# BlockstreamResearch/secp256k1-zkp

Measured on AMD Instinct MI355X. Metric: 64-bit Borromean rangeproof verifies/sec, higher is better.
Workload: dtype u32 limbs (9x29-bit), 32x32->64 integer MAC

## Files before the change

### __graft_entry__.py

```python
import os
import subprocess
import sys

ROOT = os.path.dirname(os.path.abspath(__file__))
CSRC = os.path.join(ROOT, "secp256k1_zkp_amd", "csrc")
HIPCC = os.environ.get("HIPCC", "/opt/rocm/bin/hipcc")
HIP_FLAGS = ["--offload-arch=gfx950", "-O3", "-std=c++17", "-shared", "-fPIC", "-Wno-unused-value"]


def _run(cmd, cwd=None):
    print("+", " ".join(cmd), flush=True)
    subprocess.check_call(cmd, cwd=cwd)


def _stale(target, sources):
    if not os.path.exists(target):
        return True
    t = os.path.getmtime(target)
    return any(os.path.getmtime(s) > t for s in sources if os.path.exists(s))


def build(force=False):
    hdrs = [os.path.join(CSRC, f) for f in os.listdir(CSRC) if f.endswith((".h", ".hip"))] + [os.path.join(ROOT, "include", "secp256k1_zkp_amd.h")]
    sys.path.insert(0, ROOT)
    from secp256k1_zkp_amd import build_lib
    build_lib.build(force=force)
    prims_src = os.path.join(ROOT, "tests", "gpu_prims", "prims.hip")
    prims = os.path.join(ROOT, "tests", "gpu_prims", "libs2k_gpuprims.so")
    if force or _stale(prims, hdrs + [prims_src]):
        _run([HIPCC] + HIP_FLAGS + ["-o", prims, prims_src])
    winv_src = os.path.join(ROOT, "tests", "wave_inverse", "waveinv_test.hip")
    winv = os.path.join(ROOT, "tests", "wave_inverse", "libs2k_waveinv_test.so")
    if force or _stale(winv, hdrs + [winv_src]):
        _run([HIPCC] + HIP_FLAGS + ["-o", winv, winv_src])
    wlanes_src = os.path.join(ROOT, "tests", "wave_inverse", "waveinv_lanes_test.hip")
    wlanes = os.path.join(ROOT, "tests", "wave_inverse", "libs2k_waveinv_lanes_test.so")
    if force or _stale(wlanes, hdrs + [wlanes_src]):
        _run([HIPCC] + HIP_FLAGS + ["-o", wlanes, wlanes_src])
    emu_src = os.path.join(ROOT, "tests", "host_emul", "hostemu.cpp")
    emu = os.path.join(ROOT, "tests", "host_emul", "libs2k_hostemu.so")
    if force or _stale(emu, hdrs + [emu_src]):
        _run(["g++", "-O2", "-std=c++17", "-fPIC", "-shared", "-o", emu, emu_src])
    ecdsa_emu_src = os.path.join(ROOT, "tests", "host_emul", "ecdsa_emu.cpp")
    ecdsa_emu = os.path.join(ROOT, "tests", "host_emul", "libs2k_ecdsa_emu.so")
    if force or _stale(ecdsa_emu, hdrs + [emu_src, ecdsa_emu_src]):
        _run(["g++", "-O2", "-std=c++17", "-fPIC", "-shared", "-o", ecdsa_emu, ecdsa_emu_src])
    wl_emu_src = os.path.join(ROOT, "tests", "host_emul", "whitelist_emu.cpp")
    wl_emu = os.path.join(ROOT, "tests", "host_emul", "libs2k_whitelist_emu.so")
    if force or _stale(wl_emu, hdrs + [emu_src, wl_emu_src]):
        _run(["g++", "-O2", "-std=c++17", "-fPIC", "-shared", "-o", wl_emu, wl_emu_src])
    tw_emu_src = os.path.join(ROOT, "tests", "host_emul", "tweak_emu.cpp")
    tw_emu = os.path.join(ROOT, "tests", "host_emul", "libs2k_tweak_emu.so")
    if force or _stale(tw_emu, hdrs + [emu_src, tw_emu_src]):
        _run(["g++", "-O2", "-std=c++17", "-fPIC", "-shared", "-o", tw_emu, tw_emu_src])
    gen_emu_src = os.path.join(ROOT, "tests", "host_emul", "generator_emu.cpp")
    gen_emu = os.path.join(ROOT, "tests", "host_emul", "libs2k_generator_emu.so")
    if force or _stale(gen_emu, hdrs + [emu_src, gen_emu_src]):
        _run(["g++", "-O2", "-std=c++17", "-fPIC", "-shared", "-o", gen_emu, gen_emu_src])
    ad_emu_src = os.path.join(ROOT, "tests", "host_emul", "adaptor_emu.cpp")
    ad_emu = os.path.join(ROOT, "tests", "host_emul", "libs2k_adaptor_emu.so")
    if force or _stale(ad_emu, hdrs + [emu_src, ad_emu_src]):
        _run(["g++", "-O2", "-std=c++17", "-fPIC", "-shared", "-o", ad_emu, ad_emu_src])
    mu_emu_src = os.path.join(ROOT, "tests", "host_emul", "musig_emu.cpp")
    mu_emu = os.path.join(ROOT, "tests", "host_emul", "libs2k_musig_emu.so")
    if force or _stale(mu_emu, hdrs + [emu_src, mu_emu_src]):
        _run(["g++", "-O2", "-std=c++17", "-fPIC", "-shared", "-o", mu_emu, mu_emu_src])
    rj_emu_src = os.path.join(ROOT, "tests", "host_emul", "ring_joint_emu.cpp")
    for name, flags in (("libs2k_ring_joint_emu.so", []), ("libs2k_ring_joint0_emu.so", ["-DS2K_RING_JOINT=0"])):
        rj_emu = os.path.join(ROOT, "tests", "host_emul", name)
        if force or _stale(rj_emu, hdrs + [emu_src, rj_emu_src]):
            _run(["g++", "-O2", "-std=c++17", "-fPIC", "-shared"] + flags + ["-o", rj_emu, rj_emu_src])
    r3_emu_src = os.path.join(ROOT, "tests", "host_emul", "ring_triple_emu.cpp")
    r3_emu = os.path.join(ROOT, "tests", "host_emul", "libs2k_ring_triple_emu.so")
    if force or _stale(r3_emu, hdrs + [emu_src, r3_emu_src]):
        _run(["g++", "-O2", "-std=c++17", "-fPIC", "-shared", "-o", r3_emu, r3_emu_src])
    r3_bounds_src = os.path.join(ROOT, "tests", "host_emul", "ring_triple_bounds.cpp")
    r3_bounds = os.path.join(ROOT, "tests", "host_emul", "ring_triple_bounds")
    if force or _stale(r3_bounds, hdrs + [emu_src, r3_emu_src, r3_bounds_src]):
        _run(["g++", "-O1", "-std=c++17", "-fsanitize=address,undefined", "-fno-sanitize-recover=undefined", "-static-libasan", "-static-libubsan", "-o", r3_bounds, r3_bounds_src])
    r3_prims_src = os.path.join(ROOT, "tests", "gpu_prims", "ring_triple_prims.hip")
    r3_prims = os.path.join(ROOT, "tests", "gpu_prims", "libs2k_ring_triple_prims.so")
    if force or _stale(r3_prims, hdrs + [r3_prims_src]):
        _run([HIPCC] + HIP_FLAGS + ["-o", r3_prims, r3_prims_src])
    if os.path.exists(os.path.join(ROOT, "oracle", "zkp_oracle.c")):
        _run(["make", "-s", "-C", os.path.join(ROOT, "oracle"), "oracle"])
    if os.path.isdir(os.environ.get("S2K_REFERENCE", "/root/reference")):
        _run(["make", "-s", "-C", os.path.join(ROOT, "oracle"), "ref", "hooked", "benches", "routed"])
    sys.path.insert(0, ROOT)
    import secp256k1_zkp_amd
    from secp256k1_zkp_amd import _native
    _native.load()


def smoke():
    sys.path.insert(0, ROOT)
    from tests import smoke_impl
    smoke_impl.run()


if __name__ == "__main__":
    build(force="--force" in sys.argv)
    if "--smoke" in sys.argv:
        smoke()
```

### secp256k1_zkp_amd/csrc/ecmult.h

```cpp
#pragma once
#include "group.h"
#include "scalar.h"

#ifndef S2K_GTAB_BITS
#define S2K_GTAB_BITS 26
#endif
#define S2K_GTAB_MAX_BITS 26
#define S2K_GTAB_ENTRY_WORDS 16
#define S2K_GTAB_SWORDS 9
#define S2K_GTAB_MAX_WINDOWS 32
struct gtab_geom { u32 D, W; };
S2K_HD u32 gtab_windows_for(u32 D) { return (256u + D - 1u) / D; }
S2K_HD u32 gtab_top_bits_for(u32 D) { return 256u - D * (gtab_windows_for(D) - 1u); }
S2K_HD int gtab_bits_ok(u32 D) { return D >= 8u && D <= S2K_GTAB_MAX_BITS && gtab_top_bits_for(D) >= 1u && gtab_top_bits_for(D) < D - 1u; }
S2K_HD size_t gtab_slot(u32 D, u32 w, u32 v) { return ((size_t)w << (D - 1u)) + (size_t)v; }
S2K_HD size_t gtab_slots_for(u32 D) { return gtab_slot(D, gtab_windows_for(D), 0) + 1; }
S2K_HD size_t gtab_words_for(u32 D) { return gtab_slots_for(D) * S2K_GTAB_ENTRY_WORDS; }
S2K_HD gtab_geom gtab_geometry(const u32* tab) { gtab_geom g; g.D = tab[0]; g.W = tab[1]; return g; }
S2K_HD void gtab_write_header(u32* tab, u32 D) {
    const u32 W = gtab_windows_for(D);
    tab[0] = D; tab[1] = W;
    for (int i = 0; i < S2K_GTAB_SWORDS; i++) {
        u32 k = 0;
        for (u32 w = 0; w + 1 < W; w++) { const u32 bit = D - 1u + D * w; if ((bit >> 5) == (u32)i) k |= 1u << (bit & 31u); }
// ... 359 lines not shown
        out[hf].neg = lo_neg; out[2 + hf].neg = h.neg;
    }
}
S2K_HD int ecmult_lane_split(gej& R, const gej& A, const gej& T, const scalar& na, const scalar& ng, int has_ng, const u32* gtab, const lane_mem& lm) {
    u32* const ptab = lm.ptab; const s2k_lds_ptr dig = lm.dig;
    const int p_active = (!A.inf) & (!T.inf) & (!sc_is_zero(na));
    const int g_active = has_ng & (!sc_is_zero(ng));
    if (!(S2K_WAVE_ALL(p_active) && (S2K_WAVE_ALL(g_active) || !S2K_WAVE_ANY(g_active)))) return 0;
    u32 sneg = 0;
    S2K_PROF_DECL;
    {
        half_scalar h0, h1; sc_split_lambda_odd(h0, h1, na);
        piece65 pc[4]; sc_split_pieces(pc, h0, h1);
        u32 dw[8];
#pragma unroll
        for (int i = 0; i < 8; i++) dw[i] = 0;
#pragma unroll
        for (int st = 0; st < 4; st++) {
            sneg |= (u32)pc[st].neg << st;
#pragma unroll
            for (int pos = 0; pos < 16; pos++) {
                const int i = 15 - pos, bit = 4 * i + 1, word = bit >> 5, sh = bit & 31;
                const u64 pair = (u64)pc[st].w[word] | ((u64)(word + 1 < 3 ? pc[st].w[word + 1] : 0u) << 32);
                const u32 v = (u32)(pair >> sh) & 15u;
                const int nib = pos * 4 + st;
                dw[nib >> 3] |= v << ((nib & 7) * 4);
            }
        }
#pragma unroll
        for (int i = 0; i < 8; i++) dig[i * S2K_DIG_STRIDE] = dw[i];
        {
            u32 ngr[S2K_GTAB_SWORDS]; gtab_recode(ngr, ng.d, gtab);
#pragma unroll
            for (int i = 0; i < S2K_GTAB_SWORDS; i++) dig[(8 + i) * S2K_DIG_STRIDE] = ngr[i];
        }
        fe za, zt, ziso;
        S2K_PROF_MARK(1);
        ptab_build_raw(za, ptab, A);
        ptab_build_raw(zt, ptab + S2K_PTAB_TABLE_WORDS, T);
        S2K_PROF_MARK(8);
        ptab_rescale(ptab, &zt);
        ptab_rescale(ptab + S2K_PTAB_TABLE_WORDS, &za);
        S2K_PROF_MARK(9);
        fe_mul(ziso, za, zt);
#pragma unroll
        for (int i = 0; i < 9; i++) ptab[S2K_PTAB_ZISO + i] = ziso.n[i];
    }
    const gtab_geom GG = gtab_geometry(gtab);
    const int a_g0 = S2K_SPLIT_ADDS_P;
    const int a_end = g_active ? a_g0 + (int)GG.W : a_g0;
    auto op_locate = [&](const u32*& addr, int& valid, int& neg, int& lam, int idx) {
        addr = ptab; valid = 0; neg = 0; lam = 0;
        if (idx < a_g0) {
            const int st = idx & 3;
            u32 v = 8u;
            if (idx >= 4) { const int nib = idx - 4; v = (dig[(nib >> 3) * S2K_DIG_STRIDE] >> ((nib & 7) * 4)) & 15u; }
            valid = 1;
            neg = (v < 8u) ^ (int)((sneg >> st) & 1u);
            const u32 e = (v < 8u) ? (7u - v) : (v - 8u);
            addr = ptab + (st >> 1) * S2K_PTAB_TABLE_WORDS + e * S2K_PTAB_ENTRY_WORDS + (((st & 1) && S2K_PTAB_TWINS) ? 16 : 0); lam = (st & 1) && !S2K_PTAB_TWINS;
        } else if (idx < a_end) {
            const int g = idx - a_g0, w = (int)(((u32)g * GG.D) >> 5);
            valid = gtab_locate(addr, neg, gtab, GG, g, dig[(8 + w) * S2K_DIG_STRIDE], w + 1 < S2K_GTAB_SWORDS ? dig[(9 + w) * S2K_DIG_STRIDE] : 0u);
        }
    };
    auto op_decode = [&](ge& o, const u32 raw[16], int neg, int lam) {
        fe y, yn;
        fe_from_words(o.x, raw); fe_from_words(y, raw + 8);
        if (lam) { fe beta; fe_set_beta(beta); fe_mul(o.x, o.x, beta); }
        fe_neg(yn, y, 1);
        fe_select(o.y, yn, y, neg);
    };
    const u32* nxt_addr; int nxt_valid, nxt_neg, nxt_lam;
    u32 raw[16];
    ge cur; int cur_valid;
    op_locate(nxt_addr, nxt_valid, nxt_neg, nxt_lam, 0);
#pragma unroll
    for (int k = 0; k < 16; k++) raw[k] = nxt_addr[k];
    op_decode(cur, raw, nxt_neg, 0);
    op_locate(nxt_addr, nxt_valid, nxt_neg, nxt_lam, 1);
    int au = 0;
    while (au < a_g0) {
        if (au >= 4 && !(au & 3)) {
#pragma unroll 1
            for (int k = 0; k < 4; k++) gej_double_lean(R, R);
            S2K_PROF_MARK(6);
        }
#pragma unroll
        for (int k = 0; k < 16; k++) raw[k] = nxt_addr[k];
        if (au == 0) gej_set_ge(R, cur);
        else { const int same_x = gej_add_ge_lean(R, R, cur); if (S2K_WAVE_ANY(same_x)) return 0; }
        op_decode(cur, raw, nxt_neg, !S2K_PTAB_TWINS);
        op_locate(nxt_addr, nxt_valid, nxt_neg, nxt_lam, au + 2);
#pragma unroll
        for (int k = 0; k < 16; k++) raw[k] = nxt_addr[k];
        { const int same_x = gej_add_ge_lean(R, R, cur); if (S2K_WAVE_ANY(same_x)) return 0; }
        au += 2;
        op_decode(cur, raw, nxt_neg, 0); cur_valid = nxt_valid;
        op_locate(nxt_addr, nxt_valid, nxt_neg, nxt_lam, au + 1);
    }
    { fe zi; ptab_load_ziso(zi, ptab); fe_mul(R.z, R.z, zi); }
#if S2K_XYZZ_TABLE_PART
    gez acc4; acc4.inf = 0; acc4.x = R.x; acc4.y = R.y;
    fe_sqr(acc4.zz, R.z); fe_mul(acc4.zzz, acc4.zz, R.z);
#endif
    while (au < a_end) {
#if S2K_NT_GTAB_SPLIT && defined(__HIP_DEVICE_COMPILE__)
        {
            typedef unsigned int s2k_u32x4 __attribute__((ext_vector_type(4)));
            const s2k_u32x4* q = (const s2k_u32x4*)nxt_addr;
#pragma unroll
            for (int k = 0; k < 4; k++) { const s2k_u32x4 v = __builtin_nontemporal_load(q + k); raw[4 * k] = v.x; raw[4 * k + 1] = v.y; raw[4 * k + 2] = v.z; raw[4 * k + 3] = v.w; }
        }
#else
#pragma unroll
        for (int k = 0; k < 16; k++) raw[k] = nxt_addr[k];
#endif
#if S2K_XYZZ_TABLE_PART
        {
            gez t = acc4; gez_add_ge_lean(t, cur);
            if (S2K_WAVE_ALL(cur_valid)) acc4 = t;
            else { fe_cmov(acc4.x, t.x, cur_valid); fe_cmov(acc4.y, t.y, cur_valid); fe_cmov(acc4.zz, t.zz, cur_valid); fe_cmov(acc4.zzz, t.zzz, cur_valid); }
        }
#else
        gej t; const int same_x = gej_add_ge_lean(t, R, cur);
        if (S2K_WAVE_ANY(same_x & cur_valid)) return 0;
        if (cur_valid) R = t;
#endif
        au++;
        op_decode(cur, raw, nxt_neg, nxt_lam); cur_valid = nxt_valid;
        op_locate(nxt_addr, nxt_valid, nxt_neg, nxt_lam, au + 1);
    }
#if S2K_XYZZ_TABLE_PART
    if (S2K_WAVE_ANY(fe_normalizes_to_zero(acc4.zz))) return 0;
    gej_set_gez(R, acc4);
#endif
    S2K_PROF_MARK(10);
#ifdef S2K_ON_SPLIT_DONE
    S2K_ON_SPLIT_DONE();
#endif
    return 1;
}


#ifndef S2K_RING_JOINT
#define S2K_RING_JOINT 1
#endif
#if S2K_RING_JOINT
#define S2K_RING_W 3
#define S2K_RING_DIGITS 22
#define S2K_RING_ADDS_P (2 * S2K_RING_DIGITS)
#define S2K_RING_GROUP 2
#else
#define S2K_RING_W 5
#define S2K_RING_DIGITS 13
#define S2K_RING_ADDS_P (4 * S2K_RING_DIGITS)
#define S2K_RING_GROUP 4
#endif
#define S2K_RING_ENTRIES 16
#define S2K_RING_DIG_WORDS 27
#define S2K_RTAB_TABLE_WORDS (S2K_RING_ENTRIES * 16)
#define S2K_RTAB_ZISO (2 * S2K_RTAB_TABLE_WORDS)
#define S2K_RTAB_WORDS (S2K_RTAB_ZISO + 16)
#if defined(__HIP_DEVICE_COMPILE__)
#define S2K_RAW_WS 64
#else
#define S2K_RAW_WS 1
#endif
#define S2K_RAW_ES (27 * S2K_RAW_WS)
#define S2K_RRAW_WAVE_WORDS (2 * S2K_RING_ENTRIES * 27 * 64)

S2K_HD void rraw_store(u32* raw, int w, const fe& a) {
#pragma unroll
    for (int i = 0; i < 9; i++) {
        if (S2K_NT_PARK && S2K_RAW_WS > 1) S2K_ST_NT(a.n[i], &raw[(w + i) * S2K_RAW_WS]);
        else raw[(w + i) * S2K_RAW_WS] = a.n[i];
    }
}
S2K_HD void rraw_load(fe& a, const u32* raw, int w) {
#pragma unroll
    for (int i = 0; i < 9; i++) a.n[i] = (S2K_NT_PARK && S2K_RAW_WS > 1) ? S2K_LD_NT(&raw[(w + i) * S2K_RAW_WS]) : raw[(w + i) * S2K_RAW_WS];
}
#if S2K_RING_JOINT
#define S2K_RJ_CHAIN_SLOT 24
#define S2K_RJ_PAIR0 144
#define S2K_RJ_PAIR_WORDS 45
S2K_HD u32 ring_piece_field(const piece65& p, int i) {
    const int bit = S2K_RING_W * i + 1, word = bit >> 5, sh = bit & 31;
    const u64 pair = (u64)p.w[word] | ((u64)(word + 1 < 3 ? p.w[word + 1] : 0u) << 32);
    u32 v = (u32)(pair >> sh) & 7u;
    if (i == S2K_RING_DIGITS - 1) v |= 4u;
    return v;
}
S2K_HD u32 ring_joint_field(u32 vc, u32 vt, u32 sc, u32 st) {
    const u32 neg = (u32)(vc < 4u) ^ sc;
    const u32 ai = vc < 4u ? 3u - vc : vc - 4u;
    const u32 bi = vt ^ ((neg ^ st) ? 7u : 0u);
    return (neg << 5) | (ai << 3) | bi;
}
S2K_HD void ring_joint_recode(u32 dw[9], const piece65 pc[4]) {
#pragma unroll
    for (int i = 0; i < 9; i++) dw[i] = 0;
#pragma unroll
    for (int hf = 0; hf < 2; hf++) {
#pragma unroll
        for (int pos = 0; pos < S2K_RING_DIGITS; pos++) {
            const int i = S2K_RING_DIGITS - 1 - pos, idx = pos * 2 + hf;
            const u32 v = ring_joint_field(ring_piece_field(pc[hf], i), ring_piece_field(pc[2 + hf], i), (u32)pc[hf].neg, (u32)pc[2 + hf].neg);
            dw[idx / 5] |= v << ((idx % 5) * 6);
        }
    }
}
S2K_HD void ecmult_ring_tables(u32* rtab, u32* raw, const gej& C, const gej& T) {
    {
        fe za, zt, zs;
        ptab_build_raw_n<4, S2K_RAW_WS, S2K_RAW_ES>(za, raw + S2K_RJ_CHAIN_SLOT * S2K_RAW_ES, C);
        ptab_build_raw_n<4, S2K_RAW_WS, S2K_RAW_ES>(zt, raw + (S2K_RJ_CHAIN_SLOT + 4) * S2K_RAW_ES, T);
#pragma unroll 1
        for (int e = 7; e >= 0; e--) {
            if ((e & 3) == 3) zs = (e >> 2) ? za : zt;
            fe x, y, h, zs2, zs3;
            rraw_load(x, raw, (S2K_RJ_CHAIN_SLOT + e) * 27); rraw_load(y, raw, (S2K_RJ_CHAIN_SLOT + e) * 27 + 9); rraw_load(h, raw, (S2K_RJ_CHAIN_SLOT + e) * 27 + 18);
            fe_sqr(zs2, zs); fe_mul(zs3, zs2, zs);
            fe_mul2(x, x, zs2, y, y, zs3);
            rraw_store(raw, 18 * e, x); rraw_store(raw, 18 * e + 9, y);
            fe_mul(zs, zs, h);
        }
        fe_mul(zs, za, zt);
#pragma unroll
        for (int i = 0; i < 9; i++) rtab[S2K_RTAB_ZISO + i] = zs.n[i];
    }
    {
        fe p; fe_set_int(p, 1);
#pragma unroll 1
        for (int k = 0; k < 16; k++) {
            const int w1o = 18 * (k >> 2), w2o = 18 * (4 + (k & 3)), rec = S2K_RJ_PAIR0 + S2K_RJ_PAIR_WORDS * k;
            fe x1, y1, x2, y2;
            rraw_load(x1, raw, w1o); rraw_load(y1, raw, w1o + 9); rraw_load(x2, raw, w2o); rraw_load(y2, raw, w2o + 9);
            fe dx, dy, sy, t, c, d, d2, w1, w2, e, a1, x3, x3m, y3, y3m;
            fe_neg(t, x1, 1); fe_add2(dx, x2, t); fe_norm_weak(dx);
            fe_neg(t, y1, 1); fe_add2(dy, y2, t); fe_norm_weak(dy);
            fe_add2(sy, y1, y2); fe_norm_weak(sy);
            fe_sqr2(c, dx, d, dy);
            fe_mul2(w1, x1, c, w2, x2, c);
            fe_neg(e, w1, 1); fe_add(e, w2);
            fe_mul_sqr(a1, y1, e, d2, sy);
            fe_add2(t, w1, w2); fe_neg(t, t, 2);
            fe_add2(x3, d, t); fe_add2(x3m, d2, t);
            fe_neg(t, x3, 4); fe_add(t, w1);
            fe_neg(e, w1, 1); fe_add(e, x3m);
            fe_mul2(y3, dy, t, y3m, sy, e);
            fe_neg(t, a1, 1); fe_add(y3, t); fe_add(y3m, t);
            rraw_store(raw, rec, x3); rraw_store(raw, rec + 9, y3); rraw_store(raw, rec + 18, x3m); rraw_store(raw, rec + 27, y3m);
            rraw_store(raw, rec + 36, p);
            fe_mul(p, p, dx);
        }
    }
    fe s; fe_set_int(s, 1);
#pragma unroll 1
    for (int k = 15; k >= 0; k--) {
        const int ai = k >> 2, bi = k & 3, rec = S2K_RJ_PAIR0 + S2K_RJ_PAIR_WORDS * k;
        fe xp, yp, xm, ym, m, x1, dx;
        rraw_load(xp, raw, rec); rraw_load(yp, raw, rec + 9); rraw_load(xm, raw, rec + 18); rraw_load(ym, raw, rec + 27); rraw_load(m, raw, rec + 36);
        rraw_load(x1, raw, 18 * ai); rraw_load(dx, raw, 18 * (4 + bi));
        fe_neg(x1, x1, 1); fe_add(dx, x1); fe_norm_weak(dx);
        fe_mul2(m, m, s, s, s, dx);
        fe m2, m3; fe_sqr(m2, m); fe_mul(m3, m2, m);
        fe_mul2(xp, xp, m2, xm, xm, m2);
        fe_mul2(yp, yp, m3, ym, ym, m3);
        fe_normalize(xp); fe_normalize(yp); fe_normalize(xm); fe_normalize(ym);
        u32* const ep = rtab + (ai * 8 + 4 + bi) * 16;
        u32* const em = rtab + (ai * 8 + 3 - bi) * 16;
        u32 wx[8], wy[8];
        fe_to_words(wx, xp); fe_to_words(wy, yp);
#pragma unroll
        for (int i = 0; i < 8; i++) { ep[i] = wx[i]; ep[8 + i] = wy[i]; }
        fe_to_words(wx, xm); fe_to_words(wy, ym);
#pragma unroll
        for (int i = 0; i < 8; i++) { em[i] = wx[i]; em[8 + i] = wy[i]; }
    }
    fe ziso;
#pragma unroll
    for (int i = 0; i < 9; i++) ziso.n[i] = rtab[S2K_RTAB_ZISO + i];
    fe_mul(ziso, ziso, s);
#pragma unroll
    for (int i = 0; i < 9; i++) rtab[S2K_RTAB_ZISO + i] = ziso.n[i];
}
#else
S2K_HD void ecmult_ring_tables(u32* rtab, u32* raw, const gej& C, const gej& T) {
    fe za, zt, ziso;
    u32* const raw_t = raw + S2K_RING_ENTRIES * S2K_RAW_ES;
    ptab_build_raw_n<S2K_RING_ENTRIES, S2K_RAW_WS, S2K_RAW_ES>(za, raw, C);
    ptab_build_raw_n<S2K_RING_ENTRIES, S2K_RAW_WS, S2K_RAW_ES>(zt, raw_t, T);
    ptab_rescale_n<S2K_RING_ENTRIES, S2K_RAW_WS, S2K_RAW_ES>(raw, rtab, 16, &zt);
    ptab_rescale_n<S2K_RING_ENTRIES, S2K_RAW_WS, S2K_RAW_ES>(raw_t, rtab + S2K_RTAB_TABLE_WORDS, 16, &za);
    fe_mul(ziso, za, zt);
#pragma unroll
    for (int i = 0; i < 9; i++) rtab[S2K_RTAB_ZISO + i] = ziso.n[i];
}
#endif
struct piece43 { u64 m; int neg; };
#define S2K_R3_DIGITS 22
#define S2K_R3_Q0 36
#define S2K_R3_PAIR0 180
#define S2K_R3_T0 180
#define S2K_R3_S1PAIR0 300
#define S2K_R3_CHAIN0 702
#define S2K_R3_PAIR_WORDS 45
S2K_HD void sc_split_pieces3(piece43 out[6], const half_scalar& h0, const half_scalar& h1) {
    const u64 mask = (1ull << 43) - 1ull;
    for (int hf = 0; hf < 2; hf++) {
        const half_scalar& h = hf ? h1 : h0;
        const u64 lo = (u64)h.w[0] | ((u64)h.w[1] << 32), mid = (u64)h.w[2] | ((u64)h.w[3] << 32);
        long long p0 = (long long)(lo & mask);
        long long p1 = (long long)(((lo >> 43) | (mid << 21)) & mask);
        long long p2 = (long long)((mid >> 22) | ((u64)h.w[4] << 42));
        if (!(p2 & 1)) { p2 += 1; p1 -= (long long)(1ull << 43); }
        if (!(p1 & 1)) { p1 += 1; p0 -= (long long)(1ull << 43); }
        const long long p[3] = {p0, p1, p2};
        for (int b = 0; b < 3; b++) { out[2 * b + hf].m = (u64)(p[b] < 0 ? -p[b] : p[b]); out[2 * b + hf].neg = (p[b] < 0) ^ h.neg; }
    }
}
S2K_HD u32 ring3_piece_field(u64 m, int i) { return (u32)((((m >> 1) | (1ull << 43)) >> (2 * i)) & 3ull); }
S2K_HD u32 ring3_field(u32 vc, u32 v1, u32 v2, u32 sc, u32 s1, u32 s2) {
    const u32 neg = (u32)(vc < 2u) ^ sc;
    const u32 ai = vc < 2u ? 1u - vc : vc - 2u;
    const u32 bi = v1 ^ ((neg ^ s1) ? 3u : 0u);
    const u32 ci = v2 ^ ((neg ^ s2) ? 3u : 0u);
    return (neg << 5) | (ai << 4) | (bi << 2) | ci;
}
S2K_HD void ring3_recode(u32 dw[9], const piece43 pc[6]) {
#pragma unroll
    for (int i = 0; i < 9; i++) dw[i] = 0;
#pragma unroll
    for (int hf = 0; hf < 2; hf++) {
#pragma unroll
        for (int pos = 0; pos < S2K_R3_DIGITS; pos++) {
            const int i = S2K_R3_DIGITS - 1 - pos, idx = pos * 2 + hf;
            const u32 v = ring3_field(ring3_piece_field(pc[hf].m, i), ring3_piece_field(pc[2 + hf].m, i), ring3_piece_field(pc[4 + hf].m, i),
                                      (u32)pc[hf].neg, (u32)pc[2 + hf].neg, (u32)pc[4 + hf].neg);
            dw[idx / 5] |= v << ((idx % 5) * 6);
        }
    }
}
struct ring3_pair { fe xp, yp, xm, ym, m, dx; };
S2K_HD void ring3_pair_add(ring3_pair& r, const u32* raw, int w1o, int w2o) {
    fe x1, y1, x2, y2;
    rraw_load(x1, raw, w1o); rraw_load(y1, raw, w1o + 9); rraw_load(x2, raw, w2o); rraw_load(y2, raw, w2o + 9);
    fe dy, sy, t, c, d, d2, w1, w2, e, a1;
    fe_neg(t, x1, 1); fe_add2(r.dx, x2, t); fe_norm_weak(r.dx);
    fe_neg(t, y1, 1); fe_add2(dy, y2, t); fe_norm_weak(dy);
    fe_add2(sy, y1, y2); fe_norm_weak(sy);
    fe_sqr2(c, r.dx, d, dy);
    fe_mul2(w1, x1, c, w2, x2, c);
    fe_neg(e, w1, 1); fe_add(e, w2);
    fe_mul_sqr(a1, y1, e, d2, sy);
    fe_add2(t, w1, w2); fe_neg(t, t, 2);
    fe_add2(r.xp, d, t); fe_add2(r.xm, d2, t);
    fe_neg(t, r.xp, 4); fe_add(t, w1);
    fe_neg(e, w1, 1); fe_add(e, r.xm);
    fe_mul2(r.yp, dy, t, r.ym, sy, e);
    fe_neg(t, a1, 1); fe_add(r.yp, t); fe_add(r.ym, t);
}
S2K_HD void ring3_pair_scale(ring3_pair& r, fe& s) {
    fe m;
    fe_mul2(m, r.m, s, s, s, r.dx);
    fe m2, m3; fe_sqr(m2, m); fe_mul(m3, m2, m);
    fe_mul2(r.xp, r.xp, m2, r.xm, r.xm, m2);
    fe_mul2(r.yp, r.yp, m3, r.ym, r.ym, m3);
}
template <int N, int KEEP_LAST, class W1, class W2, class Out>
S2K_HD void ring3_pair_batch(fe& s, u32* raw, int rec0, W1 w1, W2 w2, Out out) {
    ring3_pair r;
    fe p; fe_set_int(p, 1);
#pragma unroll 1
    for (int k = 0; k < N - KEEP_LAST; k++) {
        const int rec = rec0 + S2K_R3_PAIR_WORDS * k;
        ring3_pair_add(r, raw, w1(k), w2(k));
        rraw_store(raw, rec, r.xp); rraw_store(raw, rec + 9, r.yp); rraw_store(raw, rec + 18, r.xm); rraw_store(raw, rec + 27, r.ym);
        rraw_store(raw, rec + 36, p);
        fe_mul(p, p, r.dx);
    }
    fe_set_int(s, 1);
    if (KEEP_LAST) {
        ring3_pair_add(r, raw, w1(N - 1), w2(N - 1));
        r.m = p;
        ring3_pair_scale(r, s);
        out(N - 1, r);
    }
#pragma unroll 1
    for (int k = N - 1 - KEEP_LAST; k >= 0; k--) {
        const int rec = rec0 + S2K_R3_PAIR_WORDS * k;
        rraw_load(r.xp, raw, rec); rraw_load(r.yp, raw, rec + 9); rraw_load(r.xm, raw, rec + 18); rraw_load(r.ym, raw, rec + 27); rraw_load(r.m, raw, rec + 36);
        fe x1; rraw_load(x1, raw, w1(k)); rraw_load(r.dx, raw, w2(k));
        fe_neg(x1, x1, 1); fe_add(r.dx, x1); fe_norm_weak(r.dx);
        ring3_pair_scale(r, s);
        out(k, r);
    }
}
S2K_HD void ecmult_ring3_tables(u32* rtab, u32* raw, const gej& C, const gej& T1, const gej& T2) {
    {
        fe za, z1, z2, zoa, zo1, zo2, zs;
        ptab_build_raw_n<2, S2K_RAW_WS, S2K_RAW_ES>(za, raw + S2K_R3_CHAIN0 * S2K_RAW_WS, C);
        ptab_build_raw_n<2, S2K_RAW_WS, S2K_RAW_ES>(z1, raw + (S2K_R3_CHAIN0 + 54) * S2K_RAW_WS, T1);
        ptab_build_raw_n<2, S2K_RAW_WS, S2K_RAW_ES>(z2, raw + (S2K_R3_CHAIN0 + 108) * S2K_RAW_WS, T2);
        fe_mul2(zoa, z1, z2, zo1, za, z2);
        fe_mul(zo2, za, z1);
#pragma unroll 1
        for (int e = 5; e >= 0; e--) {
            if (e == 5) zs = zo2; else if (e == 3) zs = zo1; else if (e == 1) zs = zoa;
            const int src = S2K_R3_CHAIN0 + 27 * e, dst = e < 2 ? 18 * e : S2K_R3_T0 + 18 * (e - 2);
            fe x, y, h, zs2, zs3;
            rraw_load(x, raw, src); rraw_load(y, raw, src + 9); rraw_load(h, raw, src + 18);
            fe_sqr(zs2, zs); fe_mul(zs3, zs2, zs);
            fe_mul2(x, x, zs2, y, y, zs3);
            rraw_store(raw, dst, x); rraw_store(raw, dst + 9, y);
            fe_mul(zs, zs, h);
        }
        fe_mul(zs, zoa, za);
#pragma unroll
        for (int i = 0; i < 9; i++) rtab[S2K_RTAB_ZISO + i] = zs.n[i];
    }
    fe d1, d2;
    ring3_pair_batch<4, 0>(d1, raw, S2K_R3_S1PAIR0,
        [](int k) { return S2K_R3_T0 + 18 * (k >> 1); }, [](int k) { return S2K_R3_T0 + 36 + 18 * (k & 1); },
        [&](int k, const ring3_pair& r) {
            const int q = S2K_R3_Q0 + 36 * k;
            rraw_store(raw, q, r.xp); rraw_store(raw, q + 9, r.yp); rraw_store(raw, q + 18, r.xm); rraw_store(raw, q + 27, r.ym);
        });
    {
        fe m2, m3; fe_sqr(m2, d1); fe_mul(m3, m2, d1);
#pragma unroll 1
        for (int e = 0; e < 2; e++) {
            fe x, y; rraw_load(x, raw, 18 * e); rraw_load(y, raw, 18 * e + 9);
            fe_mul2(x, x, m2, y, y, m3);
            rraw_store(raw, 18 * e, x); rraw_store(raw, 18 * e + 9, y);
        }
    }
    ring3_pair_batch<16, 1>(d2, raw, S2K_R3_PAIR0,
        [](int k) { return 18 * (k >> 3); }, [](int k) { return S2K_R3_Q0 + 18 * (k & 7); },
        [&](int k, ring3_pair& r) {
            const int ai = k >> 3, bi = 2 + ((k >> 2) & 1), ca = (k >> 1) & 1, ci = (k & 1) ? 1 - ca : 2 + ca;
            fe_normalize(r.xp); fe_normalize(r.yp); fe_normalize(r.xm); fe_normalize(r.ym);
            u32* const ep = rtab + (ai * 16 + bi * 4 + ci) * 16;
            u32* const em = rtab + (ai * 16 + (3 - bi) * 4 + (3 - ci)) * 16;
            u32 wx[8], wy[8];
            fe_to_words(wx, r.xp); fe_to_words(wy, r.yp);
#pragma unroll
            for (int i = 0; i < 8; i++) { ep[i] = wx[i]; ep[8 + i] = wy[i]; }
            fe_to_words(wx, r.xm); fe_to_words(wy, r.ym);
#pragma unroll
            for (int i = 0; i < 8; i++) { em[i] = wx[i]; em[8 + i] = wy[i]; }
        });
    fe ziso;
#pragma unroll
    for (int i = 0; i < 9; i++) ziso.n[i] = rtab[S2K_RTAB_ZISO + i];
    fe_mul(d1, d1, d2); fe_mul(ziso, ziso, d1);
#pragma unroll
    for (int i = 0; i < 9; i++) rtab[S2K_RTAB_ZISO + i] = ziso.n[i];
}
S2K_HD void ring_step_recode(u32 dw[9], u32& sneg, const half_scalar& h0, const half_scalar& h1) {
    piece65 pc[4]; sc_split_pieces(pc, h0, h1);
#if S2K_RING_JOINT
    ring_joint_recode(dw, pc);
#else
#pragma unroll
    for (int i = 0; i < 9; i++) dw[i] = 0;
#pragma unroll
    for (int st = 0; st < 4; st++) {
        sneg |= (u32)pc[st].neg << st;
#pragma unroll
        for (int pos = 0; pos < S2K_RING_DIGITS; pos++) {
            const int i = S2K_RING_DIGITS - 1 - pos, bit = S2K_RING_W * i + 1, word = bit >> 5, sh = bit & 31;
            const u64 pair = (u64)pc[st].w[word] | ((u64)(word + 1 < 3 ? pc[st].w[word + 1] : 0u) << 32);
            u32 v = (u32)(pair >> sh) & 31u;
            if (pos == 0) v |= 16u;
            const int nib = pos * 4 + st;
            dw[nib / 6] |= v << ((nib % 6) * 5);
        }
    }
#endif
}
template <int TRIPLE>
S2K_HD int ecmult_ring_step_t(gej& R, const u32* rtab, const scalar& e, const scalar& s, const scalar& f, int has_f, const u32* gtab, const u32* htab,
                              const s2k_lds_ptr dig) {
    constexpr int RING_W = TRIPLE ? 2 : S2K_RING_W, RING_GROUP = TRIPLE ? 2 : S2K_RING_GROUP, RING_ADDS_P = TRIPLE ? 2 * S2K_R3_DIGITS : S2K_RING_ADDS_P;
    constexpr bool FIELDS = TRIPLE || S2K_RING_JOINT;
    u32 sneg = 0; (void)sneg;
    S2K_PROF_DECL;
    {
        half_scalar h0, h1; sc_split_lambda_odd(h0, h1, e);
        u32 dw[9];
        if constexpr (TRIPLE) { piece43 pc3[6]; sc_split_pieces3(pc3, h0, h1); ring3_recode(dw, pc3); }
        else ring_step_recode(dw, sneg, h0, h1);
#pragma unroll
        for (int i = 0; i < 9; i++) dig[i * S2K_DIG_STRIDE] = dw[i];
        u32 sr[S2K_GTAB_SWORDS], fr[S2K_GTAB_SWORDS]; gtab_recode(sr, s.d, gtab); gtab_recode(fr, f.d, has_f ? htab : gtab);
#pragma unroll
        for (int i = 0; i < S2K_GTAB_SWORDS; i++) { dig[(9 + i) * S2K_DIG_STRIDE] = sr[i]; dig[(18 + i) * S2K_DIG_STRIDE] = fr[i]; }
    }
    S2K_PROF_MARK(1);
    const gtab_geom GG = gtab_geometry(gtab), GH = gtab_geometry(has_f ? htab : gtab);
    const int a_g0 = RING_ADDS_P, a_h0 = a_g0 + (int)GG.W;
    const int a_end = has_f ? a_h0 + (int)GH.W : a_h0;
    auto op_locate = [&](const u32*& addr, int& valid, int& neg, int idx) {
        addr = rtab; valid = 0; neg = 0;
        if (idx < a_g0) {
            if constexpr (FIELDS) {
                const u32 v = (dig[(idx / 5) * S2K_DIG_STRIDE] >> ((idx % 5) * 6)) & 63u;
                valid = 1;
                neg = (int)(v >> 5);
                addr = rtab + (v & 31u) * 16;
            } else {
                const int st = idx & 3;
                const u32 v = (dig[(idx / 6) * S2K_DIG_STRIDE] >> ((idx % 6) * 5)) & 31u;
                valid = 1;
                neg = (v < 16u) ^ (int)((sneg >> st) & 1u);
                const u32 en = (v < 16u) ? (15u - v) : (v - 16u);
                addr = rtab + (st >> 1) * S2K_RTAB_TABLE_WORDS + en * 16;
            }
        } else if (idx < a_end) {
            const int second = idx >= a_h0;
            const int g = idx - (second ? a_h0 : a_g0), base = second ? 18 : 9, w = (int)(((u32)g * (second ? GH.D : GG.D)) >> 5);
            valid = gtab_locate(addr, neg, second ? htab : gtab, second ? GH : GG, g, dig[(base + w) * S2K_DIG_STRIDE], w + 1 < S2K_GTAB_SWORDS ? dig[(base + 1 + w) * S2K_DIG_STRIDE] : 0u);
        }
    };
    auto op_decode = [&](ge& o, const u32 raw[16], int neg, int lam) {
        fe y, yn;
        fe_from_words(o.x, raw); fe_from_words(y, raw + 8);
        if (lam) { fe beta; fe_set_beta(beta); fe_mul(o.x, o.x, beta); }
        fe_neg(yn, y, 1);
        fe_select(o.y, yn, y, neg);
    };
    const u32* nxt_addr; int nxt_valid, nxt_neg;
    u32 raw[16];
    ge cur; int cur_valid;
    op_locate(nxt_addr, nxt_valid, nxt_neg, 0);
#pragma unroll
    for (int k = 0; k < 16; k++) raw[k] = nxt_addr[k];
    op_decode(cur, raw, nxt_neg, 0);
    op_locate(nxt_addr, nxt_valid, nxt_neg, 1);
    int au = 0;
    while (au < a_g0) {
        if (au >= RING_GROUP && !(au & (RING_GROUP - 1))) {
            S2K_PROF_MARK(7);
#pragma unroll 1
            for (int k = 0; k < RING_W; k++) gej_double_lean(R, R);
            S2K_PROF_MARK(6);
        }
#pragma unroll
        for (int k = 0; k < 16; k++) raw[k] = nxt_addr[k];
        if (au == 0) gej_set_ge(R, cur);
        else { const int same_x = gej_add_ge_lean(R, R, cur); if (S2K_WAVE_ANY(same_x)) return 0; }
        op_decode(cur, raw, nxt_neg, 1);
        op_locate(nxt_addr, nxt_valid, nxt_neg, au + 2);
#pragma unroll
        for (int k = 0; k < 16; k++) raw[k] = nxt_addr[k];
        { const int same_x = gej_add_ge_lean(R, R, cur); if (S2K_WAVE_ANY(same_x)) return 0; }
        au += 2;
        op_decode(cur, raw, nxt_neg, 0); cur_valid = nxt_valid;
        op_locate(nxt_addr, nxt_valid, nxt_neg, au + 1);
    }
    S2K_PROF_MARK(7);
    {
        fe zi;
#pragma unroll
        for (int i = 0; i < 9; i++) zi.n[i] = rtab[S2K_RTAB_ZISO + i];
        fe_mul(R.z, R.z, zi);
#if !S2K_XYZZ_TABLE_PART
        if (FIELDS && S2K_WAVE_ANY(fe_normalizes_to_zero(zi))) return 0;
#endif
    }
#if S2K_XYZZ_TABLE_PART
    gez acc4; acc4.inf = 0; acc4.x = R.x; acc4.y = R.y;
    fe_sqr(acc4.zz, R.z); fe_mul(acc4.zzz, acc4.zz, R.z);
#endif
    while (au < a_end) {
#if S2K_NT_GTAB && defined(__HIP_DEVICE_COMPILE__)
        {
            typedef unsigned int s2k_u32x4 __attribute__((ext_vector_type(4)));
            const s2k_u32x4* q = (const s2k_u32x4*)nxt_addr;
#pragma unroll
            for (int k = 0; k < 4; k++) { const s2k_u32x4 v = __builtin_nontemporal_load(q + k); raw[4 * k] = v.x; raw[4 * k + 1] = v.y; raw[4 * k + 2] = v.z; raw[4 * k + 3] = v.w; }
        }
#else
#pragma unroll
        for (int k = 0; k < 16; k++) raw[k] = nxt_addr[k];
#endif
#if S2K_XYZZ_TABLE_PART
        {
            gez t = acc4; gez_add_ge_lean(t, cur);
            if (S2K_WAVE_ALL(cur_valid)) acc4 = t;
            else { fe_cmov(acc4.x, t.x, cur_valid); fe_cmov(acc4.y, t.y, cur_valid); fe_cmov(acc4.zz, t.zz, cur_valid); fe_cmov(acc4.zzz, t.zzz, cur_valid); }
        }
#else
        gej t; const int same_x = gej_add_ge_lean(t, R, cur);
        if (S2K_WAVE_ANY(same_x & cur_valid)) return 0;
        if (cur_valid) R = t;
#endif
        au++;
        op_decode(cur, raw, nxt_neg, 0); cur_valid = nxt_valid;
        op_locate(nxt_addr, nxt_valid, nxt_neg, au + 1);
    }
#if S2K_XYZZ_TABLE_PART
    if (S2K_WAVE_ANY(fe_normalizes_to_zero(acc4.zz))) return 0;
    gej_set_gez(R, acc4);
#endif
    S2K_PROF_MARK(10);
#ifdef S2K_ON_RING_STEP_DONE
    S2K_ON_RING_STEP_DONE();
#endif
    return 1;
}
S2K_HD int ecmult_ring_step(gej& R, const u32* rtab, const scalar& e, const scalar& s, const scalar& f, int has_f, const u32* gtab, const u32* htab,
                            const s2k_lds_ptr dig) {
    return ecmult_ring_step_t<0>(R, rtab, e, s, f, has_f, gtab, htab, dig);
}
S2K_HD int ecmult_ring3_step(gej& R, const u32* rtab, const scalar& e, const scalar& s, const scalar& f, int has_f, const u32* gtab, const u32* htab,
                             const s2k_lds_ptr dig) {
    return ecmult_ring_step_t<1>(R, rtab, e, s, f, has_f, gtab, htab, dig);
}


#define S2K_JOINT_ADDS (4 * 33)
S2K_HD int ecmult_lane2(gej& R, const gej& A, const scalar& na, const gej& B, const scalar& nb, const lane_mem& lm) {
    u32* const ptab = lm.ptab; const s2k_lds_ptr dig = lm.dig;
    const int active = (!A.inf) & (!B.inf) & (!sc_is_zero(na)) & (!sc_is_zero(nb));
    if (!S2K_WAVE_ALL(active)) return 0;
    u32 sneg = 0;
    S2K_PROF_DECL;
    {
        u32 dw[16];
#pragma unroll
        for (int i = 0; i < 16; i++) dw[i] = 0;
        auto put = [&](const half_scalar& h, const int st) {
            sneg |= (u32)h.neg << st;
#pragma unroll
            for (int pos = 0; pos < 32; pos++) {
                const int i = 31 - pos, bit = 4 * i + 1, word = bit >> 5, sh = bit & 31;
                const u64 pair = (u64)h.w[word] | ((u64)h.w[word + 1] << 32);
                const u32 v = (u32)(pair >> sh) & 15u;
                const int nib = pos * 4 + st;
                dw[nib >> 3] |= v << ((nib & 7) * 4);
            }
        };
        { half_scalar h0, h1; sc_split_lambda_odd(h0, h1, na); put(h0, 0); put(h1, 1); }
        { half_scalar h0, h1; sc_split_lambda_odd(h0, h1, nb); put(h0, 2); put(h1, 3); }
#pragma unroll
        for (int i = 0; i < 16; i++) dig[i * S2K_DIG_STRIDE] = dw[i];
        fe za, zb, ziso;
        S2K_PROF_MARK(1);
        ptab_build_raw(za, ptab, A);
        ptab_build_raw(zb, ptab + S2K_PTAB_TABLE_WORDS, B);
        fe_mul(ziso, za, zb);
        if (S2K_WAVE_ANY(fe_normalizes_to_zero(ziso))) return 0;
        S2K_PROF_MARK(8);
        ptab_rescale(ptab, &zb);
        ptab_rescale(ptab + S2K_PTAB_TABLE_WORDS, &za);
        S2K_PROF_MARK(9);
#pragma unroll
        for (int i = 0; i < 9; i++) ptab[S2K_PTAB_ZISO + i] = ziso.n[i];
    }
    auto op_locate = [&](const u32*& addr, int& neg, int idx) {
        const int st = idx & 3;
        u32 v = 8u;
        if (idx >= 4 && idx < S2K_JOINT_ADDS) { const int nib = idx - 4; v = (dig[(nib >> 3) * S2K_DIG_STRIDE] >> ((nib & 7) * 4)) & 15u; }
        neg = (v < 8u) ^ (int)((sneg >> st) & 1u);
        const u32 e = (v < 8u) ? (7u - v) : (v - 8u);
        addr = ptab + (st >> 1) * S2K_PTAB_TABLE_WORDS + e * S2K_PTAB_ENTRY_WORDS + (((st & 1) && S2K_PTAB_TWINS) ? 16 : 0);
    };
    auto op_decode = [&](ge& o, const u32 raw[16], int neg, int lam) {
        fe y, yn;
        fe_from_words(o.x, raw); fe_from_words(y, raw + 8);
        if (lam) { fe beta; fe_set_beta(beta); fe_mul(o.x, o.x, beta); }
        fe_neg(yn, y, 1);
        fe_select(o.y, yn, y, neg);
    };
    const u32* nxt_addr; int nxt_neg;
    u32 raw[16];
    ge cur;
    op_locate(nxt_addr, nxt_neg, 0);
#pragma unroll
    for (int k = 0; k < 16; k++) raw[k] = nxt_addr[k];
    op_decode(cur, raw, nxt_neg, 0);
    op_locate(nxt_addr, nxt_neg, 1);
    int au = 0;
    while (au < S2K_JOINT_ADDS) {
        if (au >= 4 && !(au & 3)) {
#pragma unroll 1
            for (int k = 0; k < 4; k++) gej_double_lean(R, R);
            S2K_PROF_MARK(6);
        }
#pragma unroll
        for (int k = 0; k < 16; k++) raw[k] = nxt_addr[k];
        if (au == 0) gej_set_ge(R, cur);
        else { const int same_x = gej_add_ge_lean(R, R, cur); if (S2K_WAVE_ANY(same_x)) return 0; }
        op_decode(cur, raw, nxt_neg, !S2K_PTAB_TWINS);
        op_locate(nxt_addr, nxt_neg, au + 2);
#pragma unroll
        for (int k = 0; k < 16; k++) raw[k] = nxt_addr[k];
        { const int same_x = gej_add_ge_lean(R, R, cur); if (S2K_WAVE_ANY(same_x)) return 0; }
        au += 2;
        op_decode(cur, raw, nxt_neg, 0);
        op_locate(nxt_addr, nxt_neg, au + 1);
    }
    { fe zi; ptab_load_ziso(zi, ptab); fe_mul(R.z, R.z, zi); }
    S2K_PROF_MARK(10);
#ifdef S2K_ON_JOINT_DONE
    S2K_ON_JOINT_DONE();
#endif
    return 1;
}

#define S2K_PARK_GEJ_WORDS 28
S2K_HD void gej_park(u32* p, size_t stride, const gej& a) {
    fe x = a.x, y = a.y, z = a.z;
    fe_norm_weak(x); fe_norm_weak(y); fe_norm_weak(z);
#pragma unroll
    for (int i = 0; i < 9; i++) { p[i * stride] = x.n[i]; p[(9 + i) * stride] = y.n[i]; p[(18 + i) * stride] = z.n[i]; }
    p[27 * stride] = (u32)a.inf;
}
S2K_HD void gej_unpark(gej& a, const u32* p, size_t stride) {
#pragma unroll
    for (int i = 0; i < 9; i++) { a.x.n[i] = p[i * stride]; a.y.n[i] = p[(9 + i) * stride]; a.z.n[i] = p[(18 + i) * stride]; }
    a.inf = (int)p[27 * stride];
}
template <class Load>
S2K_HD void ecmult_lane2_calls(gej& R, Load load, const u32* gtab, const lane_mem& lm, u32* park, size_t park_stride) {
    scalar zero; sc_set_zero(zero);
    {
        gej P, T; scalar n;
        load(0, P, n);
        ecmult_lane(T, P, n, zero, 0, gtab, lm);
        gej_park(park, park_stride, T);
    }
    gej P, T, F; scalar n;
    load(1, P, n);
    ecmult_lane(T, P, n, zero, 0, gtab, lm);
    gej_unpark(F, park, park_stride);
    gej_add_var(R, F, T);
}
S2K_HD u32 s2k_opaque_zero() { u32 z = 0; S2K_CHAIN(z); return z; }
// ... 1 lines not shown
```

Before: 1.139 million.

## Store only prefix products in ring3 pair batch and recompute pair adds backward

The ring3 pair batch previously computed each pair addition in a forward pass and parked five field elements per pair (xp, yp, xm, ym, prefix product) in scratch memory, then reloaded them in the backward pass. Now the forward pass only computes dx differences and stores prefix products, and the backward pass recomputes the full pair addition from the source points. It also prefetches the next iteration's inputs (AHEAD). This shrinks scratch footprint and memory traffic, at the cost of redundant field arithmetic.

```diff
diff --git a/__graft_entry__.py b/__graft_entry__.py
--- a/__graft_entry__.py
+++ b/__graft_entry__.py
@@ -78,6 +78,14 @@
     r3_bounds = os.path.join(ROOT, "tests", "host_emul", "ring_triple_bounds")
     if force or _stale(r3_bounds, hdrs + [emu_src, r3_emu_src, r3_bounds_src]):
         _run(["g++", "-O1", "-std=c++17", "-fsanitize=address,undefined", "-fno-sanitize-recover=undefined", "-static-libasan", "-static-libubsan", "-o", r3_bounds, r3_bounds_src])
+    r3p_emu_src = os.path.join(ROOT, "tests", "host_emul", "ring_table_prefix_emu.cpp")
+    r3p_emu = os.path.join(ROOT, "tests", "host_emul", "libs2k_ring_table_prefix_emu.so")
+    if force or _stale(r3p_emu, hdrs + [emu_src, r3_emu_src, r3p_emu_src]):
+        _run(["g++", "-O2", "-std=c++17", "-fPIC", "-shared", "-o", r3p_emu, r3p_emu_src])
+    r3p_bounds_src = os.path.join(ROOT, "tests", "host_emul", "ring_table_prefix_bounds.cpp")
+    r3p_bounds = os.path.join(ROOT, "tests", "host_emul", "ring_table_prefix_bounds")
+    if force or _stale(r3p_bounds, hdrs + [emu_src, r3_emu_src, r3p_emu_src, r3p_bounds_src]):
+        _run(["g++", "-O1", "-std=c++17", "-fsanitize=address,undefined", "-fno-sanitize-recover=undefined", "-static-libasan", "-static-libubsan", "-o", r3p_bounds, r3p_bounds_src])
     r3_prims_src = os.path.join(ROOT, "tests", "gpu_prims", "ring_triple_prims.hip")
     r3_prims = os.path.join(ROOT, "tests", "gpu_prims", "libs2k_ring_triple_prims.so")
     if force or _stale(r3_prims, hdrs + [r3_prims_src]):
diff --git a/secp256k1_zkp_amd/csrc/ecmult.h b/secp256k1_zkp_amd/csrc/ecmult.h
--- a/secp256k1_zkp_amd/csrc/ecmult.h
+++ b/secp256k1_zkp_amd/csrc/ecmult.h
@@ -685,11 +685,14 @@
 struct piece43 { u64 m; int neg; };
 #define S2K_R3_DIGITS 22
 #define S2K_R3_Q0 36
-#define S2K_R3_PAIR0 180
+#define S2K_R3_PROD0 180
 #define S2K_R3_T0 180
-#define S2K_R3_S1PAIR0 300
-#define S2K_R3_CHAIN0 702
-#define S2K_R3_PAIR_WORDS 45
+#define S2K_R3_S1PROD0 252
+#define S2K_R3_CHAIN0 252
+#define S2K_R3_PARK_WORDS 414
+#ifndef S2K_R3_AHEAD
+#define S2K_R3_AHEAD 1
+#endif
 S2K_HD void sc_split_pieces3(piece43 out[6], const half_scalar& h0, const half_scalar& h1) {
     const u64 mask = (1ull << 43) - 1ull;
     for (int hf = 0; hf < 2; hf++) {
@@ -727,9 +730,7 @@
     }
 }
 struct ring3_pair { fe xp, yp, xm, ym, m, dx; };
-S2K_HD void ring3_pair_add(ring3_pair& r, const u32* raw, int w1o, int w2o) {
-    fe x1, y1, x2, y2;
-    rraw_load(x1, raw, w1o); rraw_load(y1, raw, w1o + 9); rraw_load(x2, raw, w2o); rraw_load(y2, raw, w2o + 9);
+S2K_HD void ring3_pair_add(ring3_pair& r, const fe& x1, const fe& y1, const fe& x2, const fe& y2) {
     fe dy, sy, t, c, d, d2, w1, w2, e, a1;
     fe_neg(t, x1, 1); fe_add2(r.dx, x2, t); fe_norm_weak(r.dx);
     fe_neg(t, y1, 1); fe_add2(dy, y2, t); fe_norm_weak(dy);
@@ -752,33 +753,42 @@
     fe_mul2(r.xp, r.xp, m2, r.xm, r.xm, m2);
     fe_mul2(r.yp, r.yp, m3, r.ym, r.ym, m3);
 }
-template <int N, int KEEP_LAST, class W1, class W2, class Out>
-S2K_HD void ring3_pair_batch(fe& s, u32* raw, int rec0, W1 w1, W2 w2, Out out) {
+template <int N, int AHEAD, class W1, class W2, class Out>
+S2K_HD void ring3_pair_batch(fe& s, u32* raw, int prod0, W1 w1, W2 w2, Out out) {
+    {
+        fe p, x1, x2, nx; fe_set_int(p, 1);
+        rraw_load(x1, raw, w1(0)); rraw_load(x2, raw, w2(0));
+#pragma unroll 1
+        for (int k = 0; k < N; k++) {
+            if (k + 1 < N) rraw_load(nx, raw, w2(k + 1));
+            if (k > 0 && w1(k) != w1(k - 1)) rraw_load(x1, raw, w1(k));
+            fe dx, t;
+            fe_neg(t, x1, 1); fe_add2(dx, x2, t); fe_norm_weak(dx);
+            if (k > 0) rraw_store(raw, prod0 + 9 * (k - 1), p);
+            fe_mul(p, p, dx);
+            x2 = nx;
+        }
+    }
+    fe_set_int(s, 1);
     ring3_pair r;
-    fe p; fe_set_int(p, 1);
+    fe x1, y1, x2, y2, nx, ny, nm;
+    if (AHEAD) { rraw_load(x2, raw, w2(N - 1)); rraw_load(y2, raw, w2(N - 1) + 9); rraw_load(r.m, raw, prod0 + 9 * (N - 2)); }
 #pragma unroll 1
-    for (int k = 0; k < N - KEEP_LAST; k++) {
-        const int rec = rec0 + S2K_R3_PAIR_WORDS * k;
-        ring3_pair_add(r, raw, w1(k), w2(k));
-        rraw_store(raw, rec, r.xp); rraw_store(raw, rec + 9, r.yp); rraw_store(raw, rec + 18, r.xm); rraw_store(raw, rec + 27, r.ym);
-        rraw_store(raw, rec + 36, p);
-        fe_mul(p, p, r.dx);
-    }
-    fe_set_int(s, 1);
-    if (KEEP_LAST) {
-        ring3_pair_add(r, raw, w1(N - 1), w2(N - 1));
-        r.m = p;
-        ring3_pair_scale(r, s);
-        out(N - 1, r);
-    }
-#pragma unroll 1
-    for (int k = N - 1 - KEEP_LAST; k >= 0; k--) {
-        const int rec = rec0 + S2K_R3_PAIR_WORDS * k;
-        rraw_load(r.xp, raw, rec); rraw_load(r.yp, raw, rec + 9); rraw_load(r.xm, raw, rec + 18); rraw_load(r.ym, raw, rec + 27); rraw_load(r.m, raw, rec + 36);
-        fe x1; rraw_load(x1, raw, w1(k)); rraw_load(r.dx, raw, w2(k));
-        fe_neg(x1, x1, 1); fe_add(r.dx, x1); fe_norm_weak(r.dx);
+    for (int k = N - 1; k >= 0; k--) {
+#pragma unroll
+        for (int i = 0; i < 9; i++) S2K_OPAQUE(s.n[i]);
+        if (k == N - 1 || w1(k) != w1(k + 1)) { rraw_load(x1, raw, w1(k)); rraw_load(y1, raw, w1(k) + 9); }
+        if (AHEAD) {
+            if (k > 0) { rraw_load(nx, raw, w2(k - 1)); rraw_load(ny, raw, w2(k - 1) + 9); }
+            if (k > 1) rraw_load(nm, raw, prod0 + 9 * (k - 2)); else fe_set_int(nm, 1);
+        } else {
+            rraw_load(x2, raw, w2(k)); rraw_load(y2, raw, w2(k) + 9);
+            if (k > 0) rraw_load(r.m, raw, prod0 + 9 * (k - 1)); else fe_set_int(r.m, 1);
+        }
+        ring3_pair_add(r, x1, y1, x2, y2);
         ring3_pair_scale(r, s);
         out(k, r);
+        if (AHEAD) { x2 = nx; y2 = ny; r.m = nm; }
     }
 }
 S2K_HD void ecmult_ring3_tables(u32* rtab, u32* raw, const gej& C, const gej& T1, const gej& T2) {
@@ -805,7 +815,7 @@
         for (int i = 0; i < 9; i++) rtab[S2K_RTAB_ZISO + i] = zs.n[i];
     }
     fe d1, d2;
-    ring3_pair_batch<4, 0>(d1, raw, S2K_R3_S1PAIR0,
+    ring3_pair_batch<4, S2K_R3_AHEAD>(d1, raw, S2K_R3_S1PROD0,
         [](int k) { return S2K_R3_T0 + 18 * (k >> 1); }, [](int k) { return S2K_R3_T0 + 36 + 18 * (k & 1); },
         [&](int k, const ring3_pair& r) {
             const int q = S2K_R3_Q0 + 36 * k;
@@ -820,7 +830,7 @@
             rraw_store(raw, 18 * e, x); rraw_store(raw, 18 * e + 9, y);
         }
     }
-    ring3_pair_batch<16, 1>(d2, raw, S2K_R3_PAIR0,
+    ring3_pair_batch<16, S2K_R3_AHEAD>(d2, raw, S2K_R3_PROD0,
         [](int k) { return 18 * (k >> 3); }, [](int k) { return S2K_R3_Q0 + 18 * (k & 7); },
         [&](int k, ring3_pair& r) {
             const int ai = k >> 3, bi = 2 + ((k >> 2) & 1), ca = (k >> 1) & 1, ci = (k & 1) ? 1 - ca : 2 + ca;
```

After: 1.165 million, median of 6. +2.3%, better.
